# phantomzone-org/fhe-ram

Measured on AMD Instinct MI355X. Metric: encrypted RAM read ops/s + write ops/s at 2^18 entries; achieved HBM GB/s vs peak, higher is better.
Workload: dtype f64

## Files before the change

### fhe-ram_amd/csrc/ctx.hpp

```cpp
#pragma once
#include "../../include/fheram.h"
#include "kernels.hpp"
#include "cmux_chain.hpp"

#include <algorithm>
#include <atomic>
#include <cstdio>
#include <cstdlib>
#include <cstring>
#include <map>
#include <string>
#include <vector>

using namespace fk;

namespace {

thread_local std::string g_create_err;


struct ProfCls {
    uint64_t launches = 0, blocks = 0;
    double ms = 0.0;
    std::vector<std::pair<hipEvent_t, hipEvent_t>> pending;
};

}

inline uint64_t next_addr_id() { static std::atomic<uint64_t> n{0}; return ++n; }

struct RamState {
    bool initialized = false, state = false;
    bool memo_top = false;
    int memo_alone = 0;
    bool res_in_trtop = false;
};

struct ReadBufs {
    int cap = 0;
    int32_t *A = nullptr, *B = nullptr;
    int32_t* C = nullptr;
    int32_t *res = nullptr, *tmp = nullptr, *tmp2 = nullptr;
    double* prep = nullptr;
    int64_t *h_res = nullptr, *d_h_res = nullptr;
};

struct fheram_ctx {
    fheram_params p;
    int device = 0;
    hipStream_t stream = nullptr;
    hipStream_t stream2 = nullptr;
    hipStream_t cur = nullptr;
    hipEvent_t ev_fork = nullptr, ev_join = nullptr;
    hipEvent_t ev_xout = nullptr, ev_xin = nullptr;
    bool side_begun = false;
    bool trhi_in_C = false;
    bool tree_rotate_pending = false;
    int ws = 0, n2 = 0, n_digits = 0;
    size_t rows = 0;
    size_t rows_glob = 0;
    int shard = 0, n_shards = 1;
    std::vector<std::vector<int>> base2d;
    static constexpr int S_CT = 3, S_ADDR = 4, S_INV = 5, DNUM_CT = 3, DNUM_GGSW = 4;
    int s_evk = 4;
    size_t atk = 0;
    static constexpr size_t GLWE = (size_t)S_CT * 2 * N;
    static constexpr size_t GLWE4 = (size_t)S_ADDR * 2 * N;
    static constexpr size_t GGSW = (size_t)DNUM_CT * 2 * GLWE4;
// ... 4 lines not shown
    double* d_atk = nullptr;
    double* d_atk_inv = nullptr;
    double* d_tsk = nullptr;
    int64_t gal[LOGN];
    bool keys_loaded = false;
    int32_t* d_data = nullptr;
    int32_t* d_tree = nullptr;
    int32_t* d_scrA = nullptr;
    int32_t* d_scrB = nullptr;
    int32_t* d_scrC = nullptr;
    int32_t* d_scrD = nullptr;
    int32_t* d_res = nullptr;
    int32_t* d_tmp = nullptr;
    int32_t* d_tmp2 = nullptr;
    int32_t* d_w = nullptr;
    double* d_big = nullptr;
    double* d_big2 = nullptr;
    int limb_split = 1;
    int chain = 1;
    int chain_y = 3;
    int fine_split = 1;
    int use_graph = 0;
    int32_t* d_part = nullptr;
    int32_t* d_gat[3] = {nullptr, nullptr, nullptr};
    int nco = 0;
    int cus = 256;
    double* d_prep = nullptr;
    bool prep1_ready = false;
    int32_t* d_ggsw_tmp = nullptr;
    int32_t* d_ggsw_tmp2 = nullptr;
    int max_digits = 0;
    RamState ram;
    bool words_staged = false;
    int memo = 1;
    int tail = 1;
    int tail_ep = 1;
    int tail_test = 0;
    unsigned tail_seq = 0;
    int tail_xoff = 0;
    uint64_t tail_launches = 0;
    unsigned* h_tail_fb = nullptr;
    unsigned tail_fb_mark = 0;
    uint64_t tail_launch_mark = 0;
    unsigned* d_tail_sync = nullptr;
    int mid = 2;
    int mid_test = 0;
    unsigned mid_seq = 0;
    uint64_t mid_launches = 0, mid_launch_mark = 0;
    unsigned mid_fb_mark = 0;
    int mid_bad_windows = 0, mid_saved = 0;
    uint64_t mid_window_cts = 0, mid_disabled_count = 0;
    unsigned mid_off_ops = 0;
    unsigned* h_mid_fb = nullptr;
    unsigned* d_mid_sync[2] = {nullptr, nullptr};
    double* d_mid_big[2] = {nullptr, nullptr};
    double* d_mid_y[2] = {nullptr, nullptr};
    int pair_z = 1;
    int fuse = 1;
    bool wide = false;
    int safe = 0;
    int monitor = 1;
    unsigned* h_ro_flag = nullptr;
    int pre_inv = 1;
    uint64_t inv_id[2] = {0, 0};
    double* d_prep_inv = nullptr;
    int32_t* d_ggsw_inv = nullptr;
// ... 185 lines not shown
```

### fhe-ram_amd/csrc/fheram.hip

```cpp
#include <unistd.h>
#include <atomic>
#include "path.hpp"

extern "C" {

int fheram_params_default(fheram_params* p) {
    if (!p) return FHERAM_ERR_INVALID_ARG;
    std::memset(p, 0, sizeof(*p));
    p->log_n = 12; p->base2k = 17; p->rank = 1;
    p->k_glwe_pt = 3; p->k_glwe_ct = 51; p->k_ggsw_addr = 68; p->k_evk_trace = 68; p->k_evk_ggsw_inv = 85;
    p->word_size = 4; p->n_decomp = 4;
    p->decomp_n[0] = p->decomp_n[1] = p->decomp_n[2] = p->decomp_n[3] = 3;
    p->max_addr = (uint64_t)1 << 14;
    return FHERAM_OK;
}

const char* fheram_last_error(const fheram_ctx* c) { return c ? c->err.c_str() : g_create_err.c_str(); }

void fheram_config_default(fheram_config* cfg) {
    if (!cfg) return;
    fheram_config d{};
    d.limb_split = 1; d.fine_split = 1; d.memo = 1; d.pre_inv = 1; d.tail = 1; d.tail_test = 0; d.mid = 2; d.mid_test = 0;
    d.chain = 1; d.chain_y = 3; d.pair_z = 1; d.fuse = 1; d.graph = 0; d.safe = 0; d.nco = 0; d.tail_ep = 1; d.monitor = 1; d.reserved = 0;
    auto env = [](const char* n) { const char* v = getenv(n); return (v && v[0]) ? v[0] : '\0'; };
    if (env("FHERAM_LIMB_SPLIT") == '0') d.limb_split = 0;
    if (env("FHERAM_FINE_SPLIT") == '0') d.fine_split = 0;
    if (env("FHERAM_MEMO") == '0') d.memo = 0;
    if (env("FHERAM_PRE_INV") == '0') d.pre_inv = 0; else if (env("FHERAM_PRE_INV") == '2') d.pre_inv = 2;
    const char tl = env("FHERAM_TAIL");
    if (tl == '0') d.tail = 0;
    d.tail_test = tl == '2' ? 1 : (tl == '3' ? 2 : 0);
    const char md = env("FHERAM_MID");
    d.mid = md == '0' ? 0 : (md == '1' ? 1 : 2);
    d.mid_test = md == '2' ? 1 : 0;
    if (env("FHERAM_CHAIN") == '0') d.chain = 0;
    if (env("FHERAM_CHAIN_Y") == '0') d.chain_y = 0;
    if (env("FHERAM_PAIR_Z") == '0') d.pair_z = 0;
    if (env("FHERAM_FUSE") == '0') d.fuse = 0;
    if (env("FHERAM_GRAPH") == '1') d.graph = 1;
    if (env("FHERAM_SAFE") == '1') d.safe = 1;
    const char nc = env("FHERAM_NCO");
    d.nco = nc == '2' ? 2 : (nc == '1' ? 1 : 0);
    if (env("FHERAM_TAIL_EP") == '0') d.tail_ep = 0;
    const char mo = env("FHERAM_MONITOR");
    if (mo == '0') d.monitor = 0; else if (mo == '2') d.monitor = 2;
    *cfg = d;
}

int fheram_ctx_create(const fheram_params* p, int device, fheram_ctx** out) {
    return fheram_ctx_create_cfg(p, device, 0, 1, nullptr, out);
}
// ... 73 lines not shown
    }
    c->cur = c->stream;
    CCHK(hipEventCreateWithFlags(&c->ev_fork, hipEventDisableTiming));
    CCHK(hipEventCreateWithFlags(&c->ev_join, hipEventDisableTiming));
    CCHK(hipEventCreateWithFlags(&c->ev_xout, hipEventDisableTiming));
    CCHK(hipEventCreateWithFlags(&c->ev_xin, hipEventDisableTiming));
    CCHK(hipEventCreate(&c->t0));
    CCHK(hipEventCreate(&c->t1));
    {
        fheram_config cfg;
        if (user_cfg) cfg = *user_cfg; else fheram_config_default(&cfg);
        c->limb_split = cfg.limb_split ? 1 : 0;
        c->fine_split = cfg.fine_split ? 1 : 0;
        c->memo = cfg.memo ? 1 : 0;
        c->pre_inv = c->memo ? (cfg.pre_inv == 2 ? 2 : (cfg.pre_inv ? 1 : 0)) : 0;
        c->tail = cfg.tail ? 1 : 0;
        static std::atomic<int> serial{0};
        c->tail_xoff = ((serial++ + (int)getpid()) & 1) * (TAIL_GROUPS / 2);
        c->tail_test = cfg.tail_test < 0 ? 0 : (cfg.tail_test > 2 ? 2 : cfg.tail_test);
        c->tail_ep = cfg.tail_ep ? 1 : 0;
        c->mid = cfg.mid < 0 ? 0 : (cfg.mid > 2 ? 2 : cfg.mid);
        c->mid_test = cfg.mid_test ? 1 : 0;
        c->chain = cfg.chain ? 1 : 0;
        c->chain_y = cfg.chain_y ? 3 : 0;
        c->pair_z = cfg.pair_z ? 1 : 0;
        c->fuse = cfg.fuse ? 1 : 0;
        c->use_graph = cfg.graph ? 1 : 0;
        if (c->use_graph) c->pre_inv = 0;
        c->safe = cfg.safe ? 1 : 0;
        if (c->safe) { c->tail = 0; c->tail_test = 0; c->mid = 0; c->mid_test = 0; if (c->pre_inv == 1) c->pre_inv = 2; }
        c->monitor = cfg.monitor < 0 ? 0 : (cfg.monitor > 2 ? 2 : cfg.monitor);
        if (c->safe && c->monitor == 1) c->monitor = 2;
        c->nco = cfg.nco == 2 ? 2 : (cfg.nco == 1 ? 1 : 0);
        hipDeviceProp_t prop;
        if (hipGetDeviceProperties(&prop, device) == hipSuccess && prop.multiProcessorCount > 0) c->cus = prop.multiProcessorCount;
    }
#define LDSATTR(k) CCHK(hipFuncSetAttribute(reinterpret_cast<const void*>(k), hipFuncAttributeMaxDynamicSharedMemorySize, (int)LDS_BYTES))
    LDSATTR(k_prepare);
    LDSATTR((&k_ext_product<3, 4, 1>));
    LDSATTR((&k_ext_product<3, 4, 2>));
    LDSATTR((&k_ext_product<3, 4, 1, 1>));
    LDSATTR((&k_ext_product_fine<3, 4>));
    LDSATTR((&k_ext_product_fine<4, 5>));
    LDSATTR((&k_ext_product_chain<3, 4>));
    LDSATTR((&k_ext_product_chain_r<4>));
    LDSATTR((&k_pair_z<4>)); LDSATTR((&k_pair_z<5>));
    LDSATTR((&k_read_chain<4, 4>)); LDSATTR((&k_read_chain<5, 4>)); LDSATTR((&k_write_chain<4, 4>)); LDSATTR((&k_write_chain<5, 4>));
    LDSATTR((&k_write_chain_t<4, 4>)); LDSATTR((&k_write_chain_t<5, 4>));
    LDSATTR((&k_read_chain_w<4, 4>)); LDSATTR((&k_read_chain_w<5, 4>));
    LDSATTR((&k_read_chain_t<4, 4>)); LDSATTR((&k_read_chain_t<5, 4>));
    LDSATTR((&k_trace_tail_t<3, 4, 3>)); LDSATTR((&k_trace_tail_t<3, 5, 3>));
    LDSATTR((&k_keyswitch_chain_w<3, 4, 3, 3>)); LDSATTR((&k_keyswitch_chain_w<3, 5, 3, 3>));
    LDSATTR((&k_keyswitch_chain<3, 4, 3>));
    LDSATTR((&k_keyswitch_chain<3, 4, 3, 3>));
    LDSATTR((&k_keyswitch_chain<3, 5, 3, 3>));
    LDSATTR((&k_trace_tail<3, 4, 3>));
    LDSATTR((&k_chain_mid<false, 4, 3, 2>)); LDSATTR((&k_chain_mid<false, 5, 3, 2>)); LDSATTR((&k_chain_mid<true, 4, 3, 2>));
    LDSATTR((&k_chain_mid<false, 4, 1, 1>)); LDSATTR((&k_chain_mid<false, 5, 1, 1>));
    LDSATTR((&k_chain_mid<false, 4, 1, 2>)); LDSATTR((&k_chain_mid<false, 5, 1, 2>));
#define LDSATTR_KS4(M, SX, SK, SO) LDSATTR((&k_keyswitch<M, SX, SK, SO, 1>)); LDSATTR((&k_keyswitch<M, SX, SK, SO, 1, 1>)); LDSATTR((&k_keyswitch_fine<M, SX, SK>))
#define LDSATTR_KS(M, SX, SK, SO) LDSATTR_KS4(M, SX, SK, SO); LDSATTR((&k_keyswitch<M, SX, SK, SO, 2>))
    LDSATTR_KS(KS_AUTO, 3, 4, 3);
    LDSATTR_KS(KS_TRACE, 3, 4, 3);
    LDSATTR_KS4(KS_PAIR, 3, 4, 3);
    LDSATTR_KS(KS_ADD, 3, 4, 3);
    LDSATTR_KS(KS_SUBNEG, 3, 4, 3);
// ... 24 lines not shown
        std::memcpy(&tw[0], &mode, 8);
        std::memcpy(&tw[N + 1], &flag_addr, 8);
    }
    CCHK(hipMalloc(&c->d_tw, TW_GLOBAL * sizeof(double)));
    CCHK(hipMemcpy(c->d_tw, tw.data(), TW_GLOBAL * sizeof(double), hipMemcpyHostToDevice));
    const size_t G = fheram_ctx::GLWE, nrow = (size_t)c->ws * c->rows;
    CCHK(hipMalloc(&c->d_atk, (size_t)LOGN * c->atk * sizeof(double)));
    CCHK(hipMalloc(&c->d_atk_inv, fheram_ctx::EVK5 * sizeof(double)));
    CCHK(hipMalloc(&c->d_tsk, fheram_ctx::EVK5 * sizeof(double)));
    CCHK(hipMalloc(&c->d_data, nrow * G * sizeof(int32_t)));
    CCHK(hipMalloc(&c->d_scrA, nrow * G * sizeof(int32_t)));
    CCHK(hipMalloc(&c->d_scrB, nrow * G * sizeof(int32_t)));
    CCHK(hipMalloc(&c->d_scrC, nrow * G * sizeof(int32_t)));
    CCHK(hipMalloc(&c->d_scrD, nrow * G * sizeof(int32_t)));
    CCHK(hipMalloc(&c->d_ggsw_tmp2, (size_t)c->max_digits * fheram_ctx::GGSW * sizeof(int32_t)));
    CCHK(hipMalloc(&c->d_tmp2, (size_t)c->ws * G * sizeof(int32_t)));
    CCHK(hipMalloc(&c->d_part, (size_t)c->ws * G * sizeof(int32_t)));
    CCHK(hipMalloc(&c->d_big, (size_t)LIMB_SPLIT_MAX * BIG_STRIDE * sizeof(double)));
    CCHK(hipMalloc(&c->d_big2, (size_t)LIMB_SPLIT_MAX * BIG_STRIDE * sizeof(double)));
    if (n_shards > 1) for (int i = 0; i < 3; i++) CCHK(hipMalloc(&c->d_gat[i], (size_t)n_shards * c->ws * G * sizeof(int32_t)));
    CCHK(hipMalloc(&c->d_tree, (size_t)c->ws * G * sizeof(int32_t)));
    CCHK(hipMalloc(&c->d_res, (size_t)c->ws * G * sizeof(int32_t)));
    CCHK(hipMalloc(&c->d_tmp, (size_t)c->ws * G * sizeof(int32_t)));
    CCHK(hipMalloc(&c->d_w, (size_t)c->ws * G * sizeof(int32_t)));
    CCHK(hipMalloc(&c->d_trtop, (size_t)c->ws * G * sizeof(int32_t)));
    CCHK(hipMalloc(&c->d_prep, (size_t)std::max(c->n_digits, c->max_digits) * fheram_ctx::GGSW * sizeof(double)));
    CCHK(hipMalloc(&c->d_ggsw_tmp, (size_t)c->max_digits * fheram_ctx::GGSW * sizeof(int32_t)));
    CCHK(hipMemset(c->d_tree, 0, (size_t)c->ws * G * sizeof(int32_t)));
    CCHK(hipMalloc(&c->d_prep_inv, (size_t)c->n_digits * fheram_ctx::GGSW * sizeof(double)));
    CCHK(hipMalloc(&c->d_ggsw_inv, (size_t)c->n_digits * fheram_ctx::GGSW * sizeof(int32_t)));
    for (int i = 0; i < 2; i++) CCHK(hipEventCreateWithFlags(&c->ev_inv[i], hipEventDisableTiming));
    CCHK(hipEventCreateWithFlags(&c->ev_wdone, hipEventDisableTiming));
    CCHK(hipEventCreateWithFlags(&c->ev_opstart, hipEventDisableTiming));
    CCHK(hipMalloc(&c->d_tail_sync, (size_t)(TAIL_GROUPS + 1) * 32 * sizeof(unsigned)));
    CCHK(hipMemset(c->d_tail_sync, 0, (size_t)(TAIL_GROUPS + 1) * 32 * sizeof(unsigned)));
    for (int i = 0; i < 2; i++) {
        CCHK(hipMalloc(&c->d_mid_sync[i], (size_t)(MID_GROUPS_MAX + 1) * 32 * sizeof(unsigned)));
        CCHK(hipMemset(c->d_mid_sync[i], 0, (size_t)(MID_GROUPS_MAX + 1) * 32 * sizeof(unsigned)));
        CCHK(hipMalloc(&c->d_mid_y[i], (size_t)2 * MID_GROUPS_MAX * 2 * N * sizeof(double)));
        CCHK(hipMalloc(&c->d_mid_big[i], (size_t)2 * MID_GROUPS_MAX * BIG_STRIDE * sizeof(double)));
    }
    CCHK(hipHostMalloc((void**)&c->h_tail_fb, 64, hipHostMallocDefault));
    *c->h_tail_fb = 0;
    CCHK(hipHostMalloc((void**)&c->h_mid_fb, 128, hipHostMallocDefault));
    memset(c->h_mid_fb, 0, 128);
    CCHK(hipHostMalloc((void**)&c->h_res, ((size_t)c->ws * G + 1) * sizeof(int64_t), hipHostMallocMapped));
    CCHK(hipHostGetDevicePointer((void**)&c->d_h_res, c->h_res, 0));
    CCHK(hipHostMalloc((void**)&c->h_w, (size_t)c->ws * G * sizeof(int32_t), hipHostMallocDefault));
    CCHK(hipEventCreateWithFlags(&c->ev_w, hipEventDisableTiming));
#undef CCHK
    *out = c;
    return FHERAM_OK;
}

void fheram_ctx_destroy(fheram_ctx* c) {
    if (!c) return;
    hipSetDevice(c->device);
    if (c->stream) hipStreamSynchronize(c->stream);
    if (c->stream2) hipStreamSynchronize(c->stream2);
    prof_collect(c);
    reads_free(c->batch);
    if (c->ev_fork) hipEventDestroy(c->ev_fork);
    if (c->ev_join) hipEventDestroy(c->ev_join);
    for (int i = 0; i < 2; i++) if (c->ev_inv[i]) hipEventDestroy(c->ev_inv[i]);
    if (c->ev_wdone) hipEventDestroy(c->ev_wdone);
    if (c->ev_opstart) hipEventDestroy(c->ev_opstart);
    if (c->ev_xout) hipEventDestroy(c->ev_xout);
    if (c->ev_xin) hipEventDestroy(c->ev_xin);
    if (c->stream2) hipStreamDestroy(c->stream2);
    for (auto e : c->ev_pool) hipEventDestroy(e);
    if (c->t0) hipEventDestroy(c->t0);
    if (c->t1) hipEventDestroy(c->t1);
    for (int b = 0; b < 2; b++) { if (c->ev_pin[b]) hipEventDestroy(c->ev_pin[b]); if (c->h_pin[b]) hipHostFree(c->h_pin[b]); }
    void* bufs[] = {c->d_tw, c->d_atk, c->d_atk_inv, c->d_tsk, c->d_data, c->d_scrA, c->d_scrB, c->d_big, c->d_big2, c->d_scrC, c->d_scrD, c->d_ggsw_tmp2, c->d_tmp2, c->d_part, c->d_gat[0], c->d_gat[1], c->d_gat[2], c->d_tree, c->d_res, c->d_tmp, c->d_w, c->d_trtop, c->d_prep, c->d_ggsw_tmp, c->d_tail_sync, c->d_prep_inv, c->d_ggsw_inv, c->d_mid_sync[0], c->d_mid_sync[1], c->d_mid_y[0], c->d_mid_y[1], c->d_mid_big[0], c->d_mid_big[1]};
    for (void* b : bufs) if (b) hipFree(b);
    if (c->h_tail_fb) hipHostFree(c->h_tail_fb);
    if (c->h_mid_fb) hipHostFree(c->h_mid_fb);
    if (c->h_res) hipHostFree(c->h_res);
    if (c->h_ro_flag) hipHostFree(c->h_ro_flag);
    if (c->h_w) hipHostFree(c->h_w);
    if (c->ev_w) hipEventDestroy(c->ev_w);
    if (c->stream) hipStreamDestroy(c->stream);
    delete c;
}

int fheram_ctx_config(const fheram_ctx* c, fheram_config* out) {
    if (!c || !out) return FHERAM_ERR_INVALID_ARG;
    fheram_config d{};
    d.limb_split = c->limb_split; d.fine_split = c->fine_split; d.memo = c->memo; d.pre_inv = c->pre_inv; d.tail = c->tail; d.tail_test = c->tail_test;
    d.mid = c->mid; d.mid_test = c->mid_test; d.chain = c->chain; d.chain_y = c->chain_y; d.pair_z = c->pair_z; d.fuse = c->fuse;
    d.graph = c->use_graph; d.safe = c->safe; d.nco = c->nco; d.monitor = c->monitor; d.tail_ep = c->tail_ep;
    *out = d;
    return FHERAM_OK;
}

size_t fheram_glwe_len(const fheram_ctx*) { return fheram_ctx::GLWE; }
size_t fheram_ggsw_len(const fheram_ctx*) { return fheram_ctx::GGSW; }
size_t fheram_atk_len(const fheram_ctx* c) { return c ? c->atk : 0; }
size_t fheram_evk_inv_len(const fheram_ctx*) { return fheram_ctx::EVK5; }
// ... 5 lines not shown
                     const int64_t* atk_ggsw_inv, int64_t atk_ggsw_inv_p, const int64_t* tsk) {
    if (!c) return FHERAM_ERR_INVALID_ARG;
    if (!gal_els || !atk_glwe || !atk_ggsw_inv || !tsk) return fail(c, FHERAM_ERR_INVALID_ARG, "null key pointer");
    if (n_gal != LOGN) return fail(c, FHERAM_ERR_KEYS, "expected log2(N) trace keys (keys.rs:39)");
    if (atk_ggsw_inv_p != -1) return fail(c, FHERAM_ERR_KEYS, "auto_key.p() != -1 (coordinate_prepared.rs:134)");
    HIPCHK(c, hipSetDevice(c->device));
    HIPCHK(c, hipStreamSynchronize(c->stream));
    HIPCHK(c, hipStreamSynchronize(c->stream2));
    int order[LOGN];
    for (int i = 0; i < LOGN; i++) {
        order[i] = -1;
        for (int j = 0; j < n_gal; j++) if (gal_els[j] == c->gal[i]) order[i] = j;
        if (order[i] < 0) return fail(c, FHERAM_ERR_KEYS, "missing trace key for a Galois element of GLWE::trace_galois_elements");
    }
    int32_t* d_stage = nullptr;
    const size_t stage_n = std::max(c->atk, fheram_ctx::EVK5);
    HIPCHK(c, hipMalloc(&d_stage, stage_n * sizeof(int32_t)));
    int rc = FHERAM_OK;
    for (int i = 0; i < LOGN && rc == FHERAM_OK; i++) {
        rc = upload_i64(c, d_stage, atk_glwe[order[i]], c->atk);
        if (rc == FHERAM_OK) launch_prepare(c, d_stage, c->d_atk + (size_t)i * c->atk, (int)(c->atk / N), c->gal[i]);
        hipStreamSynchronize(c->stream);
    }
    if (rc == FHERAM_OK) rc = upload_i64(c, d_stage, atk_ggsw_inv, fheram_ctx::EVK5);
    if (rc == FHERAM_OK) { launch_prepare(c, d_stage, c->d_atk_inv, (int)(fheram_ctx::EVK5 / N), -1); hipStreamSynchronize(c->stream); }
    if (rc == FHERAM_OK) rc = upload_i64(c, d_stage, tsk, fheram_ctx::EVK5);
    if (rc == FHERAM_OK) { launch_prepare(c, d_stage, c->d_tsk, (int)(fheram_ctx::EVK5 / N)); hipStreamSynchronize(c->stream); }
    hipFree(d_stage);
    if (rc != FHERAM_OK) return rc;
    HIPCHK(c, hipGetLastError());
    c->keys_loaded = true;
    c->inv_id[0] = c->inv_id[1] = 0;
    c->inv_pending[0] = c->inv_pending[1] = false;
    c->ram.memo_top = false; c->ram.memo_alone = 0;
    return FHERAM_OK;
}

int fheram_ram_upload(fheram_ctx* c, const int64_t* rows) {
    if (!c) return FHERAM_ERR_INVALID_ARG;
    if (!rows) return fail(c, FHERAM_ERR_INVALID_ARG, "null rows");
    HIPCHK(c, hipSetDevice(c->device));
    int rc = upload_i64(c, c->d_data, rows, (size_t)c->ws * c->rows * fheram_ctx::GLWE);
    if (rc != FHERAM_OK) return rc;
    c->ram.initialized = true; c->ram.state = false; c->ram.memo_top = false; c->ram.memo_alone = 0;
    return FHERAM_OK;
}
int fheram_ram_download(fheram_ctx* c, int64_t* rows) {
    if (!c || !rows) return FHERAM_ERR_INVALID_ARG;
    if (!c->ram.initialized) return fail(c, FHERAM_ERR_UNINITIALIZED, "unitialized memory: self.data.len()=0");
    HIPCHK(c, hipSetDevice(c->device));
    const int rc = download_i64(c, rows, c->d_data, (size_t)c->ws * c->rows * fheram_ctx::GLWE);
    return rc == FHERAM_OK ? check_precision(c) : rc;
}
int fheram_ram_tree_download(fheram_ctx* c, int level, int64_t* out) {
    if (!c || !out) return FHERAM_ERR_INVALID_ARG;
    if (level != 0 || c->n2 < 2) return fail(c, FHERAM_ERR_INVALID_ARG, "tree level does not exist (ram.rs:315-324)");
    HIPCHK(c, hipSetDevice(c->device));
    return download_i64(c, out, c->d_tree, (size_t)c->ws * fheram_ctx::GLWE);
}
int fheram_ram_state(const fheram_ctx* c) { return c ? (int)c->ram.state : 0; }

int fheram_address_create(fheram_ctx* c, const int64_t* const* ggsw, int n_ggsw, fheram_addr** out) {
    if (!c || !out) return FHERAM_ERR_INVALID_ARG;
    *out = nullptr;
    if (!ggsw) return fail(c, FHERAM_ERR_INVALID_ARG, "null ggsw");
    if (n_ggsw != c->n_digits) return fail(c, FHERAM_ERR_INVALID_ARG, "address digit count does not match the context's Base2D (ram.rs:404)");
    HIPCHK(c, hipSetDevice(c->device));
    fheram_addr* a = new fheram_addr{c, nullptr, n_ggsw, c->device};
    hipError_t e = hipMalloc(&a->d_ggsw, (size_t)n_ggsw * fheram_ctx::GGSW * sizeof(int32_t));
    if (e != hipSuccess) { delete a; return fail(c, FHERAM_ERR_DEVICE, std::string("hipMalloc: ") + hipGetErrorString(e)); }
    for (int i = 0; i < n_ggsw; i++) {
        if (!ggsw[i]) { fheram_address_destroy(a); return fail(c, FHERAM_ERR_INVALID_ARG, "null ggsw digit"); }
        int rc = upload_i64(c, a->d_ggsw + (size_t)i * fheram_ctx::GGSW, ggsw[i], fheram_ctx::GGSW);
        if (rc != FHERAM_OK) { fheram_address_destroy(a); return rc; }
    }
    *out = a;
    return FHERAM_OK;
// ... 64 lines not shown
int fheram_read_batch(fheram_ctx* c, const fheram_addr* const* addrs, int n_addr, int64_t* out) {
    if (!c) return FHERAM_ERR_INVALID_ARG;
    if (!addrs) return fail(c, FHERAM_ERR_INVALID_ARG, "null address list");
    if (n_addr < 1 || n_addr > FHERAM_READ_BATCH_MAX)
        return fail(c, FHERAM_ERR_INVALID_ARG, "n_addr = " + std::to_string(n_addr) + " is outside [1, FHERAM_READ_BATCH_MAX = " + std::to_string(FHERAM_READ_BATCH_MAX) + "]");
    for (int k = 0; k < n_addr; k++) {
        const int rc = check_common(c, addrs[k]);
        if (rc != FHERAM_OK) return rc;
    }
    if (c->n_shards != 1) return fail(c, FHERAM_ERR_INVALID_ARG, "row-sharded context: use fheram_read_partial / fheram_read_finish");
    if (c->ram.state) return fail(c, FHERAM_ERR_STATE, "invalid call to Memory.read: internal state is true -> requires calling Memory.write");
    HIPCHK(c, hipSetDevice(c->device));
    int rc;
    if (n_addr == 1) {
        rc = run_op(c, addrs[0], 0, [&] { return read_impl(one_addr(c, addrs), ctx_view(c), false); });
        if (rc != FHERAM_OK) return rc;
        HIPCHK(c, hipGetLastError());
        return out ? fheram_result_download(c, out) : FHERAM_OK;
    }
    return read_many(c, c->batch, &c->ram, addrs, n_addr, c->ws, 0, false, out, [&](const Opnds& o) {
        launch_copy(c, o.slice(ref(c->batch.res, (long)fheram_ctx::GLWE, 0), n_addr - 1), ref(c->d_res, (long)fheram_ctx::GLWE, 0), 1, c->ws);
    });
}
int fheram_read_prepare_write(fheram_ctx* c, const fheram_addr* addr, int64_t* out) {
    int rc = check_common(c, addr);
    if (rc != FHERAM_OK) return rc;
    if (c->n_shards != 1) return fail(c, FHERAM_ERR_INVALID_ARG, "row-sharded context: use fheram_read_partial / fheram_read_finish");
    if (c->ram.state) return fail(c, FHERAM_ERR_STATE, "invalid call to Memory.read: internal state is true -> requires calling Memory.write");
    HIPCHK(c, hipSetDevice(c->device));
    rc = run_op(c, addr, 1, [&] { return read_impl(one_addr(c, &addr), ctx_view(c), true); });
    if (rc != FHERAM_OK) return rc;
    c->ram.state = true;
    HIPCHK(c, hipGetLastError());
    return out ? fheram_result_download(c, out) : FHERAM_OK;
}
int fheram_word_stage(fheram_ctx* c, const int64_t* w, int n_w) {
    if (!c || !w) return FHERAM_ERR_INVALID_ARG;
    if (n_w != c->ws) return fail(c, FHERAM_ERR_INVALID_ARG, "w.len() != subrams.len() (ram.rs:243)");
    HIPCHK(c, hipSetDevice(c->device));
    const int rc = stage_words(c, c->d_w, w, c->ws);
    if (rc == FHERAM_OK) c->words_staged = true;
    return rc;
}
int fheram_write(fheram_ctx* c, const int64_t* w, int n_w, const fheram_addr* addr) {
    int rc = check_common(c, addr);
    if (rc != FHERAM_OK) return rc;
    if (n_w != c->ws) return fail(c, FHERAM_ERR_INVALID_ARG, "w.len() != subrams.len() (ram.rs:243)");
    if (!c->ram.state) return fail(c, FHERAM_ERR_STATE, "invalid call to Memory.write: internal state is false -> requires calling Memory.read_prepare_write");
    HIPCHK(c, hipSetDevice(c->device));
    if (c->n_shards != 1) return fail(c, FHERAM_ERR_INVALID_ARG, "row-sharded context: use fheram_write_root / fheram_write_shard");
    if (!w && !c->words_staged) return fail(c, FHERAM_ERR_INVALID_ARG, "w == NULL and no staged words");
    const Opnds o = one_addr(c, &addr);
    if (w && !c->side_begun && !(c->use_graph && !c->profile)) write_side_begin(o, ctx_view(c));
    if (w) { rc = fheram_word_stage(c, w, n_w); if (rc != FHERAM_OK) { write_side_abort(c); return rc; } }
    rc = run_op(c, addr, 2, [&] {
        if (!c->side_begun) write_side_begin(o, ctx_view(c));
        int r2 = write_top(o, ctx_view(c));
        return r2 == FHERAM_OK ? write_rows(o, ctx_view(c)) : r2;
    });
    if (rc != FHERAM_OK) return rc;
    c->ram.state = false;
    HIPCHK(c, hipGetLastError());
    return FHERAM_OK;
}

namespace {
int export_glwes(fheram_ctx* c, const int32_t* src, void* dst, int on_device, size_t n_glwe) {
// ... 364 lines not shown
```

### fhe-ram_amd/csrc/path.hpp

```cpp
#pragma once
#include "launch.hpp"

namespace {

struct Opnds {
    fheram_ctx* c;
    RamState* st;
    const fheram_addr* const* addrs;
    int n, ws;
    double *tab, *tab_inv;
    long stride;
    unsigned src_map;
    bool bank;
    int member(int k) const { return (int)((src_map >> (4 * k)) & 15u); }
    int Y() const { return n * ws; }
    double* prep(int k, int ci) const { return digits_of(c, tab + k * stride, ci); }
    double* inv(int k, int ci) const { return digits_of(c, tab_inv + k * stride, ci); }
    GlweRef slice(GlweRef r, int k) const { r.p += (long)k * ws * r.sy; return r; }
    GlweRef rows(GlweRef r, int k) const { return slice(r, member(k)); }
    OpndTable table() const { return n == 1 ? OpndTable{} : OpndTable{ws, stride, src_map}; }
    bool row_fuse(int d, int n_tr, int gx) const { return use_row_fuse(c, d, n_tr, gx, Y(), bank); }
};
Opnds one_addr(fheram_ctx* c, const fheram_addr* const* a, int ws, RamState* st) { return Opnds{c, st, a, 1, ws, c->d_prep, c->d_prep_inv, 0, 0, false}; }
Opnds one_addr(fheram_ctx* c, const fheram_addr* const* a) { return one_addr(c, a, c->ws, &c->ram); }
Opnds table_opnds(fheram_ctx* c, RamState* st, const fheram_addr* const* addrs, int n, int ws, double* tab, double* tab_inv, unsigned src_map, bool bank) {
    return Opnds{c, st, addrs, n, ws, tab, tab_inv, (long)c->n_digits * (long)fheram_ctx::GGSW, src_map, bank};
}

struct RamView {
    int32_t *rows, *A, *B, *C, *D;
    int32_t *part, *tmp, *tmp2, *res, *tree, *w, *trtop;
};
RamView ctx_view(const fheram_ctx* c) {
    return RamView{c->d_data, c->d_scrA, c->d_scrB, c->d_scrC, c->d_scrD, c->d_part, c->d_tmp, c->d_tmp2, c->d_res, c->d_tree, c->d_w, c->d_trtop};
}

void read_local_done(const fheram_ctx* c, RamState* st, bool prepare_write) {
    if (c->n2 == 2) st->memo_alone = (prepare_write && c->memo) ? LOGN - ilog2_ceil(c->rows_glob) : 0;
}
void read_top_done(fheram_ctx* c, RamState* st, bool prepare_write) {
    st->memo_top = prepare_write && c->memo;
    st->res_in_trtop = st->memo_top;
    c->prep1_ready = false;
}
void write_done(fheram_ctx* c, RamState* st) { st->memo_top = false; st->memo_alone = 0; c->side_begun = false; c->tree_rotate_pending = false; }

template <typename F>
int run_op(fheram_ctx* c, const fheram_addr* addr, int which, F&& enqueue) {
    if (!c->use_graph || c->profile) return enqueue();
    fheram_addr* a = const_cast<fheram_addr*>(addr);
    const unsigned sig = 1u | (c->ram.memo_top ? 2u : 0u) | ((unsigned)c->ram.memo_alone << 2) | (c->side_begun ? 64u : 0u) |
                         (c->inv_id[0] == addr->id ? 128u : 0u) | (c->inv_id[1] == addr->id ? 256u : 0u);
    if (a->graph[which] && a->graph_sig[which] != sig) { hipGraphExecDestroy(a->graph[which]); a->graph[which] = nullptr; }
    if (!a->graph[which]) {
        hipGraph_t g = nullptr;
        HIPCHK(c, hipStreamBeginCapture(c->stream, hipStreamCaptureModeThreadLocal));
        const int rc = enqueue();
        const hipError_t e = hipStreamEndCapture(c->stream, &g);
        if (rc != FHERAM_OK || e != hipSuccess) {
            if (g) hipGraphDestroy(g);
            return rc != FHERAM_OK ? rc : fail(c, FHERAM_ERR_DEVICE, std::string("hipStreamEndCapture: ") + hipGetErrorString(e));
        }
        const hipError_t e2 = hipGraphInstantiate(&a->graph[which], g, nullptr, nullptr, 0);
        hipGraphDestroy(g);
        if (e2 != hipSuccess) { a->graph[which] = nullptr; return fail(c, FHERAM_ERR_DEVICE, std::string("hipGraphInstantiate: ") + hipGetErrorString(e2)); }
        a->graph_sig[which] = sig;
    }
    HIPCHK(c, hipGraphLaunch(a->graph[which], c->stream));
    if (which == 2) write_done(c, &c->ram);
    else { read_local_done(c, &c->ram, which == 1); read_top_done(c, &c->ram, which == 1); }
    return FHERAM_OK;
}

int check_common(fheram_ctx* c, const fheram_addr* addr) {
    if (!c) return FHERAM_ERR_INVALID_ARG;
    mid_rearm(c);
    if (!addr || addr->ctx != c) return fail(c, FHERAM_ERR_INVALID_ARG, "address does not belong to this context (layout mismatch, ram.rs:404)");
    if (addr->empty) return fail(c, FHERAM_ERR_INVALID_ARG, "empty address: fheram_address_alloc without fheram_address_derive");
// ... 189 lines not shown
    GlweRef wref = ref(v.w, G, 0), tmp = ref(v.tmp, G, 0), tmp2 = ref(v.tmp2, G, 0), tree = ref(v.tree, G, 0);
    GlweRef top = (c->n2 != 1) ? tree : ref(v.rows, sy, 0);
    GlweRef tr = tmp;
    if (o.st->memo_top) tr = ref(v.trtop, G, 0);
    else trace_steps(c, top, tmp, tmp2, 0, LOGN, 1, Y);
    {
        ProfScope ps(c, "elementwise", Y);
        hipLaunchKernelGGL((k_sub_add_norm<3>), dim3(1, Y, EW_SLICES), dim3(256), 0, c->cur, top, tr, wref, top);
    }
    o.st->memo_top = false;
    if (c->n2 == 2) {
        if (n == 1 && c->inv_id[1] == o.addrs[0]->id) wait_inverse(c, c->stream, 1);
        else {
            if (n == 1 && c->inv_pending[1]) wait_inverse(c, c->stream, 1);
            for (int k = 0; k < n; k++) coordinate_prepare_inv(c, o.addrs[k], 1, c->d_ggsw_tmp, o.inv(k, 1));
        }
        if (n == 1) { c->inv_pending[1] = false; c->inv_id[1] = 0; }
        for (int k = 0; k < n; k++)
            ep_chain(c, o.slice(tree, k), o.slice(ref(v.part, G, 0), k), o.slice(tmp, k), o.inv(k, 1), (int)c->base2d[1].size(), 1, ws);
        c->tree_rotate_pending = true;
    }
    return FHERAM_OK;
}
void write_side_begin(const Opnds& o, const RamView& v) {
    fheram_ctx* c = o.c;
    c->wide = true;
    const long G = (long)fheram_ctx::GLWE;
    const long sy = (long)c->rows * G;
    hipEventRecord(c->ev_fork, c->stream);
    hipStreamWaitEvent(c->stream2, c->ev_fork, 0);
    c->cur = c->stream2;
    if (c->n2 == 2) {
        const int kept = o.st->memo_alone;
        c->trhi_in_C = kept > 0 && (LOGN - kept) % 2 == 1;
        if (kept > 0) trace_steps(c, ref(v.A, sy, G), ref(c->trhi_in_C ? v.C : v.A, sy, G), ref(c->trhi_in_C ? v.A : v.C, sy, G), kept, LOGN, (int)c->rows, o.Y());
        else trace_steps(c, ref(v.rows, sy, G), ref(v.A, sy, G), ref(v.C, sy, G), 0, LOGN, (int)c->rows, o.Y());
        o.st->memo_alone = 0;
    }
    if (o.n == 1 && c->inv_id[0] == o.addrs[0]->id) wait_inverse(c, c->stream2, 0);
    else for (int k = 0; k < o.n; k++) coordinate_prepare_inv(c, o.addrs[k], 0, c->d_ggsw_tmp2, o.inv(k, 0));
    if (o.n == 1) { c->inv_id[0] = 0; c->inv_pending[0] = false; }
    hipEventRecord(c->ev_join, c->stream2);
    c->cur = c->stream;
    c->side_begun = true;
}
void write_side_abort(fheram_ctx* c) {
    if (!c->side_begun) return;
    hipStreamWaitEvent(c->stream, c->ev_join, 0);
    c->side_begun = false;
}
int write_rows(const Opnds& o, const RamView& v) {
    fheram_ctx* c = o.c;
    c->wide = true;
    const long G = (long)fheram_ctx::GLWE;
    const long sy = (long)c->rows * G;
    const int n = o.n, ws = o.ws, Y = o.Y(), R = (int)c->rows;
    GlweRef data = ref(v.rows, sy, G), A = ref(v.A, sy, G), B = ref(v.B, sy, G), D = ref(v.D, sy, G);
    GlweRef trhi = ref(c->trhi_in_C ? v.C : v.A, sy, G), part = ref(v.part, G, 0);
    const int d0 = (int)c->base2d[0].size();
    const bool fuse = c->n2 == 2 && o.row_fuse(d0, LOGN, R);
    if (fuse) {
        hipStreamWaitEvent(c->stream, c->ev_join, 0);
        launch_write_chain(c, part, c->n_shards, c->shard, data, trhi, o.inv(0, 0), d0, LOGN, R, Y, o.table());
    } else if (c->n2 == 2)
        trace_steps(c, part, B, D, 0, LOGN, R, Y, c->n_shards, c->shard);
    if (c->tree_rotate_pending) {
        ProfScope ps(c, "elementwise", Y);
        hipLaunchKernelGGL((k_rotate<3>), dim3(1, Y, EW_SLICES), dim3(256), 0, c->cur, part, ref(v.tree, G, 0), -(int)c->rows_glob);
    }
    if (!fuse) {
        hipStreamWaitEvent(c->stream, c->ev_join, 0);
        if (c->n2 == 2) {
            ProfScope ps(c, "elementwise", (uint64_t)R * Y);
            hipLaunchKernelGGL((k_sub_add_norm<3>), dim3(R, Y, EW_SLICES), dim3(256), 0, c->cur, data, trhi, B, data);
        }
        for (int k = 0; k < n; k++) ep_chain(c, o.slice(data, k), o.slice(data, k), o.slice(A, k), o.inv(k, 0), d0, R, ws);
    }
// ... 8 lines not shown
```

### fhe-ram_amd/csrc/setup.hpp

```cpp
#pragma once
#include "launch.hpp"

namespace {
void wipe_free(hipStream_t st, void* d, size_t bytes) {
    if (!d) return;
    if (hipMemsetAsync(d, 0, bytes, st) == hipSuccess) hipStreamSynchronize(st);
    hipFree(d);
}
void wipe_host(void* p, size_t bytes) {
    volatile unsigned char* v = static_cast<volatile unsigned char*>(p);
    for (size_t i = 0; i < bytes; i++) v[i] = 0;
}
}

namespace {

constexpr int64_t NOISE_LIM = (int64_t)1 << 30;
int noise_limb(int k) { return (k + BASE2K - 1) / BASE2K - 1; }

template <int S, int DEC>
void launch_enc(fheram_ctx* c, int32_t* cts, const double* s_hat, const int32_t* pt1, int n) {
    ProfScope ps(c, "encrypt", (uint64_t)n);
    hipLaunchKernelGGL((k_encrypt_sk<S, DEC>), dim3(n), dim3(T), LDS_BYTES, c->cur, cts, s_hat, c->d_tw, pt1);
}
// ... 161 lines not shown
    if (data_len % ws != 0) return fail(c, FHERAM_ERR_INVALID_ARG, "invalid data: data.len()%ram_chunks != 0");
    if (data_len / ws != c->p.max_addr) return fail(c, FHERAM_ERR_INVALID_ARG, "invalid data: data.len()/ram_chunks != max_addr");
    const int k = (int)c->p.k_glwe_ct, S = fheram_ctx::S_CT;
    int rc = check_setup_args(c, sk, S, k);
    if (rc != FHERAM_OK) return rc;
    const int k_pt = (int)c->p.k_glwe_pt, size_pt = (k_pt + BASE2K - 1) / BASE2K;
    if (k_pt <= 0 || k_pt > 8 + BASE2K || size_pt > S) return fail(c, FHERAM_ERR_UNSUPPORTED, "k_glwe_pt out of range");
    HIPCHK(c, hipSetDevice(c->device));
    const size_t G = fheram_ctx::GLWE, max_addr = c->p.max_addr;
    const size_t CH = 256;
    std::vector<int32_t> pre(std::min(CH, c->rows) * G);
    int32_t limbs[4];
    for (size_t w = 0; w < ws; w++)
        for (size_t x0 = 0; x0 < c->rows; x0 += CH) {
            const size_t nx = std::min(CH, c->rows - x0);
            std::fill(pre.begin(), pre.begin() + nx * G, 0);
            for (size_t x = 0; x < nx; x++) {
                const size_t r = (size_t)c->shard + (x0 + x) * (size_t)c->n_shards;
                int32_t* pg = pre.data() + x * G;
                for (size_t q = 0; q < (size_t)N; q++) {
                    const size_t a = r * N + q;
                    if (a >= max_addr) break;
                    encode_value((int64_t)(int8_t)data[a * ws + w], k_pt, size_pt, limbs);
                    for (int j = 0; j < size_pt; j++) pg[(size_t)(j * 2) * N + q] = limbs[j];
                }
                const size_t gi = w * c->rows + x0 + x;
                if (!stage_random(pg, S, k, mask + gi * S * N, noise + gi * N))
                    return fail(c, FHERAM_ERR_RANGE, "mask limb outside [-2^16, 2^16) or |noise| >= 2^30");
            }
            rc = encrypt_staged(c, sk->d_hat, c->d_data + (w * c->rows + x0) * G, pre, nullptr, (int)nx, S);
            if (rc != FHERAM_OK) return rc;
        }
    c->ram.initialized = true; c->ram.state = false;
    return FHERAM_OK;
}

int fheram_address_encrypt_sk(fheram_ctx* c, const fheram_secret* sk, uint32_t value, const int64_t* mask,
                              const int64_t* noise, fheram_addr** out) {
    if (!c || !out) return FHERAM_ERR_INVALID_ARG;
    *out = nullptr;
    if (!mask || !noise) return fail(c, FHERAM_ERR_INVALID_ARG, "null argument");
    const int S = fheram_ctx::S_ADDR, k = (int)c->p.k_ggsw_addr, D = fheram_ctx::DNUM_CT;
    int rc = check_setup_args(c, sk, S, k);
    if (rc != FHERAM_OK) return rc;
    HIPCHK(c, hipSetDevice(c->device));
    {
        unsigned bits = 0;
        for (auto& b1 : c->base2d) for (int b : b1) bits += (unsigned)b;
        if (bits < 32 && ((uint64_t)value >> bits) != 0)
            return fail(c, FHERAM_ERR_INVALID_ARG, "self.base2d.max() > value (address.rs:98): address does not fit the digit plan");
    }
    const size_t glen = fheram_ctx::GLWE4;
    const int n = c->n_digits * D * 2;
    std::vector<int32_t> pre((size_t)n * glen, 0), pt1((size_t)n * S * N, 0);
    size_t remain = value;
    int gi = 0;
    for (auto& base1d : c->base2d) {
        unsigned tot = 0;
        for (int b : base1d) tot += (unsigned)b;
        const size_t max = (size_t)1 << tot;
        size_t rem_c = remain & (max - 1);
        remain /= max;
        const bool neg = rem_c != 0;
        unsigned tot_base = 0;
        for (int b : base1d) {
            const size_t chunk = (rem_c & (((size_t)1 << b) - 1)) << tot_base;
// ... 62 lines not shown
    };
    auto automorphism_key = [&](int64_t p, int rows, int S, int k, double* d_prepared, int64_t* std_dst) -> int {
        host_automorphism(galois_inv_mod(galois_mod(p)), sk->sk.data(), sk_out.data());
        hipMemcpyAsync(d_small, sk_out.data(), N * sizeof(int32_t), hipMemcpyHostToDevice, c->stream);
        launch_prepare(c, d_small, d_hat, 1);
        hipStreamSynchronize(c->stream);
        return gglwe(sk->sk.data(), d_hat, rows, S, k, d_prepared, std_dst, p);
    };
    for (int i = 0; i < LOGN && rc == FHERAM_OK; i++)
        rc = automorphism_key(c->gal[i], fheram_ctx::DNUM_CT, c->s_evk, (int)c->p.k_evk_trace,
                              c->d_atk + (size_t)i * c->atk, std_out ? std_out + (size_t)i * c->atk : nullptr);
    if (rc == FHERAM_OK) {
        std::copy(sk->sk.begin(), sk->sk.end(), ss.begin() + N);
        hipMemcpyAsync(d_small, ss.data(), 2 * N * sizeof(int32_t), hipMemcpyHostToDevice, c->stream);
        launch_enc_dyn(c, 1, 1, d_small, sk->d_hat, nullptr, 1);
        hipMemcpyAsync(ss.data(), d_small, N * sizeof(int32_t), hipMemcpyDeviceToHost, c->stream);
        if (hipStreamSynchronize(c->stream) != hipSuccess) rc = fail(c, FHERAM_ERR_DEVICE, "tensor key: s*s failed");
    }
    if (rc == FHERAM_OK)
        rc = gglwe(ss.data(), sk->d_hat, fheram_ctx::DNUM_GGSW, fheram_ctx::S_INV, (int)c->p.k_evk_ggsw_inv, c->d_tsk,
                   std_out ? std_out + (size_t)LOGN * c->atk : nullptr, 0);
    if (rc == FHERAM_OK)
        rc = automorphism_key(-1, fheram_ctx::DNUM_GGSW, fheram_ctx::S_INV, (int)c->p.k_evk_ggsw_inv, c->d_atk_inv,
                              std_out ? std_out + (size_t)LOGN * c->atk + fheram_ctx::EVK5 : nullptr);
    hipFree(d_stage);
    wipe_free(c->stream, d_small, 2 * N * sizeof(int32_t));
    wipe_free(c->stream, d_hat, N * sizeof(double));
    wipe_host(sk_out.data(), sk_out.size() * sizeof(sk_out[0])); wipe_host(ss.data(), ss.size() * sizeof(ss[0]));
    if (rc != FHERAM_OK) return rc;
    HIPCHK(c, hipGetLastError());
    c->keys_loaded = true;
    c->inv_id[0] = c->inv_id[1] = 0;
    c->inv_pending[0] = c->inv_pending[1] = false;
    c->ram.memo_top = false; c->ram.memo_alone = 0;
    return FHERAM_OK;
}

size_t fheram_fheuint_ggsw_len(const fheram_ctx*) { return fheram_ctx::GGSW5; }
namespace {
int fheuint_alloc(fheram_ctx* c, int n_bits, fheram_fheuint** out) {
    fheram_fheuint* f = new fheram_fheuint{c, c->device, n_bits, nullptr, nullptr};
    hipError_t e = hipMalloc(&f->d_std, (size_t)n_bits * fheram_ctx::GGSW5 * sizeof(int32_t));
    if (e == hipSuccess) e = hipMalloc(&f->d_prep, (size_t)n_bits * fheram_ctx::GGSW5 * sizeof(double));
    if (e != hipSuccess) { fheram_fheuint_destroy(f); return fail(c, FHERAM_ERR_DEVICE, std::string("hipMalloc: ") + hipGetErrorString(e)); }
    *out = f;
    return FHERAM_OK;
}
int fheuint_prepare(fheram_ctx* c, fheram_fheuint* f) {
    c->cur = c->stream;
    launch_prepare(c, f->d_std, f->d_prep, f->n_bits * (int)(fheram_ctx::GGSW5 / N));
    HIPCHK(c, hipStreamSynchronize(c->stream));
    HIPCHK(c, hipGetLastError());
    return FHERAM_OK;
}
}
int fheram_fheuint_create(fheram_ctx* c, const int64_t* bits, int n_bits, fheram_fheuint** out) {
    if (!c || !out) return FHERAM_ERR_INVALID_ARG;
    *out = nullptr;
    if (!bits || n_bits <= 0 || n_bits > 64) return fail(c, FHERAM_ERR_INVALID_ARG, "bad argument");
    HIPCHK(c, hipSetDevice(c->device));
    fheram_fheuint* f = nullptr;
    int rc = fheuint_alloc(c, n_bits, &f);
    if (rc == FHERAM_OK) rc = upload_i64(c, f->d_std, bits, (size_t)n_bits * fheram_ctx::GGSW5);
    if (rc == FHERAM_OK) rc = fheuint_prepare(c, f);
    if (rc != FHERAM_OK) { fheram_fheuint_destroy(f); return rc; }
    *out = f;
    return FHERAM_OK;
// ... 170 lines not shown
```

Baseline: 1308.

## Prerun remaining high trace steps on side stream after read completes

After a read finishes, the remaining memoized trace steps for the upper tree levels are launched early on the second stream, so they overlap with host-side work and the next operation's setup instead of running inside the next write's side path. A new state flag records that the steps were precomputed and which buffer holds the output, and the write path skips recomputing them. Every state reset (key load, RAM upload, encrypt, write completion) waits on the new event. The cost is extra cross-stream synchronisation and possible contention when the next operation's kernels start while the prerun is still executing.

```diff
diff --git a/fhe-ram_amd/csrc/ctx.hpp b/fhe-ram_amd/csrc/ctx.hpp
--- a/fhe-ram_amd/csrc/ctx.hpp
+++ b/fhe-ram_amd/csrc/ctx.hpp
@@ -34,6 +34,7 @@
     bool memo_top = false;
     int memo_alone = 0;
     bool res_in_trtop = false;
+    int trhi_pre = 0;
 };
 
 struct ReadBufs {
@@ -104,6 +105,8 @@
     int max_digits = 0;
     RamState ram;
     bool words_staged = false;
+    int pre_trhi = 1;
+    hipEvent_t ev_trhi = nullptr;
     int memo = 1;
     int tail = 1;
     int tail_ep = 1;
diff --git a/fhe-ram_amd/csrc/fheram.hip b/fhe-ram_amd/csrc/fheram.hip
--- a/fhe-ram_amd/csrc/fheram.hip
+++ b/fhe-ram_amd/csrc/fheram.hip
@@ -17,6 +17,7 @@
 
 const char* fheram_last_error(const fheram_ctx* c) { return c ? c->err.c_str() : g_create_err.c_str(); }
 
+static int env_pre_trhi() { const char* v = getenv("FHERAM_PRE_TRHI"); return (v && v[0] == '0') ? 0 : ((v && v[0] == '2') ? 2 : 1); }
 void fheram_config_default(fheram_config* cfg) {
     if (!cfg) return;
     fheram_config d{};
@@ -156,6 +157,7 @@
         c->monitor = cfg.monitor < 0 ? 0 : (cfg.monitor > 2 ? 2 : cfg.monitor);
         if (c->safe && c->monitor == 1) c->monitor = 2;
         c->nco = cfg.nco == 2 ? 2 : (cfg.nco == 1 ? 1 : 0);
+        c->pre_trhi = c->memo ? env_pre_trhi() : 0;
         hipDeviceProp_t prop;
         if (hipGetDeviceProperties(&prop, device) == hipSuccess && prop.multiProcessorCount > 0) c->cus = prop.multiProcessorCount;
     }
@@ -246,6 +248,7 @@
     for (int i = 0; i < 2; i++) CCHK(hipEventCreateWithFlags(&c->ev_inv[i], hipEventDisableTiming));
     CCHK(hipEventCreateWithFlags(&c->ev_wdone, hipEventDisableTiming));
     CCHK(hipEventCreateWithFlags(&c->ev_opstart, hipEventDisableTiming));
+    CCHK(hipEventCreateWithFlags(&c->ev_trhi, hipEventDisableTiming));
     CCHK(hipMalloc(&c->d_tail_sync, (size_t)(TAIL_GROUPS + 1) * 32 * sizeof(unsigned)));
     CCHK(hipMemset(c->d_tail_sync, 0, (size_t)(TAIL_GROUPS + 1) * 32 * sizeof(unsigned)));
     for (int i = 0; i < 2; i++) {
@@ -279,6 +282,7 @@
     for (int i = 0; i < 2; i++) if (c->ev_inv[i]) hipEventDestroy(c->ev_inv[i]);
     if (c->ev_wdone) hipEventDestroy(c->ev_wdone);
     if (c->ev_opstart) hipEventDestroy(c->ev_opstart);
+    if (c->ev_trhi) hipEventDestroy(c->ev_trhi);
     if (c->ev_xout) hipEventDestroy(c->ev_xout);
     if (c->ev_xin) hipEventDestroy(c->ev_xin);
     if (c->stream2) hipStreamDestroy(c->stream2);
@@ -350,7 +354,7 @@
     c->keys_loaded = true;
     c->inv_id[0] = c->inv_id[1] = 0;
     c->inv_pending[0] = c->inv_pending[1] = false;
-    c->ram.memo_top = false; c->ram.memo_alone = 0;
+    c->ram.memo_top = false; c->ram.memo_alone = 0; trhi_void(c, &c->ram);
     return FHERAM_OK;
 }
 
@@ -361,6 +365,7 @@
     int rc = upload_i64(c, c->d_data, rows, (size_t)c->ws * c->rows * fheram_ctx::GLWE);
     if (rc != FHERAM_OK) return rc;
     c->ram.initialized = true; c->ram.state = false; c->ram.memo_top = false; c->ram.memo_alone = 0;
+    trhi_void(c, &c->ram);
     return FHERAM_OK;
 }
 int fheram_ram_download(fheram_ctx* c, int64_t* rows) {
@@ -491,7 +496,10 @@
     if (rc != FHERAM_OK) return rc;
     c->ram.state = true;
     HIPCHK(c, hipGetLastError());
-    return out ? fheram_result_download(c, out) : FHERAM_OK;
+    if (out) { rc = fheram_result_download(c, out); if (rc != FHERAM_OK) return rc; }
+    prerun_trhi(one_addr(c, &addr), ctx_view(c));
+    HIPCHK(c, hipGetLastError());
+    return FHERAM_OK;
 }
 int fheram_word_stage(fheram_ctx* c, const int64_t* w, int n_w) {
     if (!c || !w) return FHERAM_ERR_INVALID_ARG;
diff --git a/fhe-ram_amd/csrc/path.hpp b/fhe-ram_amd/csrc/path.hpp
--- a/fhe-ram_amd/csrc/path.hpp
+++ b/fhe-ram_amd/csrc/path.hpp
@@ -43,7 +43,12 @@
     st->res_in_trtop = st->memo_top;
     c->prep1_ready = false;
 }
-void write_done(fheram_ctx* c, RamState* st) { st->memo_top = false; st->memo_alone = 0; c->side_begun = false; c->tree_rotate_pending = false; }
+void trhi_void(fheram_ctx* c, RamState* st) {
+    if (!st->trhi_pre) return;
+    hipStreamWaitEvent(c->stream, c->ev_trhi, 0);
+    st->trhi_pre = 0;
+}
+void write_done(fheram_ctx* c, RamState* st) { st->memo_top = false; st->memo_alone = 0; trhi_void(c, st); c->side_begun = false; c->tree_rotate_pending = false; }
 
 template <typename F>
 int run_op(fheram_ctx* c, const fheram_addr* addr, int which, F&& enqueue) {
@@ -299,8 +304,10 @@
     c->cur = c->stream2;
     if (c->n2 == 2) {
         const int kept = o.st->memo_alone;
-        c->trhi_in_C = kept > 0 && (LOGN - kept) % 2 == 1;
-        if (kept > 0) trace_steps(c, ref(v.A, sy, G), ref(c->trhi_in_C ? v.C : v.A, sy, G), ref(c->trhi_in_C ? v.A : v.C, sy, G), kept, LOGN, (int)c->rows, o.Y());
+        if (o.st->trhi_pre) c->trhi_in_C = o.st->trhi_pre == 2;
+        else c->trhi_in_C = kept > 0 && (LOGN - kept) % 2 == 1;
+        if (o.st->trhi_pre) o.st->trhi_pre = 0;
+        else if (kept > 0) trace_steps(c, ref(v.A, sy, G), ref(c->trhi_in_C ? v.C : v.A, sy, G), ref(c->trhi_in_C ? v.A : v.C, sy, G), kept, LOGN, (int)c->rows, o.Y());
         else trace_steps(c, ref(v.rows, sy, G), ref(v.A, sy, G), ref(v.C, sy, G), 0, LOGN, (int)c->rows, o.Y());
         o.st->memo_alone = 0;
     }
@@ -310,6 +317,30 @@
     hipEventRecord(c->ev_join, c->stream2);
     c->cur = c->stream;
     c->side_begun = true;
+}
+bool prerun_trhi(const Opnds& o, const RamView& v) {
+    fheram_ctx* c = o.c;
+    const int kept = o.st->memo_alone, R = (int)c->rows, Y = o.Y();
+    if (!c->pre_trhi || o.n != 1 || o.st != &c->ram || c->n2 != 2 || c->n_shards != 1 || kept <= 0 || c->use_graph || (long)R * Y > c->cus) return false;
+    c->cur = c->stream2;
+    const ChainForm form = chain_form(c, ChainQuery{false, LOGN - kept, R, Y}).form;
+    c->cur = c->stream;
+    if (form != ChainForm::Chain && form != ChainForm::Steps) return false;
+    const long G = (long)fheram_ctx::GLWE;
+    const long sy = (long)c->rows * G;
+    hipEventRecord(c->ev_fork, c->stream);
+    hipStreamWaitEvent(c->stream2, c->ev_fork, 0);
+    const bool wide = c->wide;
+    c->wide = c->pre_trhi == 2;
+    c->cur = c->stream2;
+    const bool in_C = (LOGN - kept) % 2 == 1;
+    trace_steps(c, ref(v.A, sy, G), ref(in_C ? v.C : v.A, sy, G), ref(in_C ? v.A : v.C, sy, G), kept, LOGN, R, Y);
+    hipEventRecord(c->ev_trhi, c->stream2);
+    c->cur = c->stream;
+    c->wide = wide;
+    o.st->memo_alone = 0;
+    o.st->trhi_pre = in_C ? 2 : 1;
+    return true;
 }
 void write_side_abort(fheram_ctx* c) {
     if (!c->side_begun) return;
diff --git a/fhe-ram_amd/csrc/setup.hpp b/fhe-ram_amd/csrc/setup.hpp
--- a/fhe-ram_amd/csrc/setup.hpp
+++ b/fhe-ram_amd/csrc/setup.hpp
@@ -217,6 +217,7 @@
             if (rc != FHERAM_OK) return rc;
         }
     c->ram.initialized = true; c->ram.state = false;
+    trhi_void(c, &c->ram);
     return FHERAM_OK;
 }
 
@@ -345,7 +346,7 @@
     c->keys_loaded = true;
     c->inv_id[0] = c->inv_id[1] = 0;
     c->inv_pending[0] = c->inv_pending[1] = false;
-    c->ram.memo_top = false; c->ram.memo_alone = 0;
+    c->ram.memo_top = false; c->ram.memo_alone = 0; trhi_void(c, &c->ram);
     return FHERAM_OK;
 }
 
```

Result: no change. 1311, median of 3 (+0.2%).
